# mantasu/face-crop-plus

Measured on AMD Instinct MI355X. Metric: faces/sec end-to-end (detect+align+crop), higher is better.
Workload: dtype f16x3; 1 GPU; RetinaFace detect + 5-pt align/crop, batch=32/GPU synthetic 1024x1024 RGB, strategy=largest, det_threshold=0.6, output 256x256, detector on 2 HIP streams x 16 images; global_batch=32, image_size=1024, parallelism=dp1

## Files before the change

face-crop-plus_amd/_native.py:

```python
from __future__ import annotations

import ctypes as C
import os

_HERE = os.path.dirname(os.path.abspath(__file__))
LIB_PATH = os.path.join(_HERE, "csrc", "libfcp_hip.so")
ABI_VERSION = 15

c_f32p = C.c_void_p
_lib = None


class ConvDesc(C.Structure):
    _fields_ = [
        ("in_", C.c_void_p), ("w", C.c_void_p), ("bias", C.c_void_p), ("out", C.c_void_p),
        ("res1", C.c_void_p), ("res2", C.c_void_p), ("wscale", C.c_void_p), ("in2", C.c_void_p),
        ("n", C.c_int32), ("in_h", C.c_int32), ("in_w", C.c_int32),
        ("cin", C.c_int32), ("in_ld", C.c_int32), ("in_up2", C.c_int32),
        ("cout", C.c_int32), ("kh", C.c_int32), ("kw", C.c_int32),
        ("stride", C.c_int32), ("pad", C.c_int32),
        ("out_h", C.c_int32), ("out_w", C.c_int32), ("out_ld", C.c_int32),
        ("tile_n", C.c_int32), ("cin4", C.c_int32),
        ("act_slope", C.c_float), ("alpha", C.c_float), ("alpha2", C.c_float),
        ("res1_pre", C.c_int32), ("res1_ld", C.c_int32), ("res1_h", C.c_int32),
# ... 5 lines not shown
    ]


CONV_FLAT_ADDR = 1
CONV_BALANCE_TAIL = 2
CHAIN_OUT_EVEN_ONLY = 1


class ChainDesc(C.Structure):
    _fields_ = [(k, C.c_void_p) for k in ("t1", "w2", "ws2", "b2", "w3", "ws3", "b3", "res", "out", "w1n", "ws1n",
                                          "b1n", "t1n", "t1b")] + \
               [(k, C.c_int32) for k in ("n", "h", "w", "c", "cn", "t1_ld", "res_ld", "out_ld", "t1n_ld", "nout", "tile_m", "flags",
                                         "cb", "t1b_ld", "t1b_h", "t1b_w", "t1b_stride")]


_P, _I, _F, _L = C.c_void_p, C.c_int, C.c_float, C.c_int64
SIGNATURES = {
    "fcp_conv2d_nhwc_f32": [C.POINTER(ConvDesc), _P],
    "fcp_bottleneck_chain_f16x3": [C.POINTER(ChainDesc), _P],
    "fcp_u8_to_nhwc4_f32": [_P, _P, _L, C.POINTER(C.c_float), _F, _P],
    "fcp_f32nchw_to_nhwc4_f32": [_P, _P, _I, _I, _I, C.POINTER(C.c_float), _F, _P],
    "fcp_maxpool3x3s2_nhwc_f32": [_P, _P, _I, _I, _I, _I, _I, _I, _I, _P],
    "fcp_maxpool3x3s2_split32": [_P, _P, _I, _I, _I, _I, _I, _I, _I, _P],
    "fcp_stem7x7s2_relu_pool_u8": [_P, _I, _I, _I, C.POINTER(C.c_int32), _P, _P, _P, _P, _I, _I, _P],
    "fcp_stem7x7s2_relu_pool_conv1_u8": [_P, _I, _I, _I, C.POINTER(C.c_int32), _P, _P, _P, _P, _I, _I, _P, _P, _P, _P, _I, _P],
    "fcp_stem7x7s2_relu_pool_f32": [_P, _I, _I, _I, _P, _P, _P, _P, _I, _I, _P],
    "fcp_f32_to_split32": [_P, _P, _L, _I, _P],
    "fcp_split32_to_f32": [_P, _P, _L, _I, _P],
    "fcp_absmax_nhwc": [_P, _L, _I, _I, _I, _P, _P],
    "fcp_retina_decode": [_P, _P, _P, _I, _I, _I, _F, _F, _F, _P, _P, _P, _P, _P, _P, _P, _P, _P],
    "fcp_retina_nms_select": [_P, _P, _P, _I, _I, _F, _I, _P, _P, _P, _P, _P, _P],
    "fcp_retina_gather_faces": [_P, _P, _P, _I, _I, _P, _I, _P, _P, _P, _P],
    "fcp_estimate_transform": [_P, _P, _I, _I, _I, _P, _P, _P],
    "fcp_estimate_transform_counted": [_P, _P, _I, _I, _I, _P, _P, _P, _P, _P],
# ... 116 lines not shown
```

face-crop-plus_amd/csrc/fcp_bneck_chain.hip:

```cpp
#include "fcp_conv_common.h"

#include <type_traits>

using namespace fcp_conv;

namespace {

constexpr int FCP_CHAIN_STORE_AUX = 2;

struct ChainK {
  const float* t1;  unsigned t1_bytes;  int t1_ld;
  const float* w2;  unsigned w2_bytes;  const float* ws2;  const float* b2;
  const float* w3;  unsigned w3_bytes;  const float* ws3;  const float* b3;
  const float* res; int res_ld;
  float* out;       int out_ld;    unsigned out_bytes;
  const float* w1n; unsigned w1n_bytes; const float* ws1n; const float* b1n;
  float* t1n;       int t1n_ld;
  int n, h, w, M;
  int nt_store;
  int out_even;
  const float* t1b; unsigned t1b_bytes; int t1b_ld, hb, wb, sb;
};

constexpr int BMT = 128;
// ... 2 lines not shown
constexpr int STAGE = (BMT + C) * ROWB;
constexpr int CT_OFF = 0;
constexpr int W1B_OFF = BMT * 128;
constexpr bool w1_double(int cn, bool has_c2) { return !has_c2 || W1B_OFF + 2 * cn * 128 + 2 * C * 128 <= 2 * STAGE; }
constexpr int w3b_off(int cn, bool has_c2) { return W1B_OFF + (w1_double(cn, has_c2) ? 2 : 1) * cn * 128; }
constexpr int r0_bytes(int cw, int cn, bool has_c2) { return has_c2 ? 2 * STAGE : w3b_off(cn, has_c2) + 2 * cw * 128; }
constexpr bool alias_t2(bool has_c2) { return !has_c2; }
constexpr int lds_bytes(int cw, int cn, bool has_c2, bool direct = false) {
  const int r0 = r0_bytes(cw, cn, has_c2), t2 = BMT * cw * 4;
  if (direct) return r0;
  return !alias_t2(has_c2) ? r0 + t2 : (r0 > W1B_OFF + t2 ? r0 : W1B_OFF + t2);
}
constexpr int wgs_per_cu(int cw, int cn, bool has_c2, bool direct = false) {
  if (direct) return cn == 0 && lds_bytes(cw, cn, has_c2, true) <= 80 * 1024 ? 2 : 1;
  return lds_bytes(cw, cn, has_c2) <= 80 * 1024 ? 2 : 1;
}

__device__ __forceinline__ void mfma3(f32x16& acc, const f16x8& ah, const f16x8& al, const f16x8& bh, const f16x8& bl) {
  acc = __builtin_amdgcn_mfma_f32_32x32x16_f16(al, bh, acc, 0, 0, 0);
  acc = __builtin_amdgcn_mfma_f32_32x32x16_f16(ah, bl, acc, 0, 0, 0);
  acc = __builtin_amdgcn_mfma_f32_32x32x16_f16(ah, bh, acc, 0, 0, 0);
}

__device__ __forceinline__ void row_values8(const float* c8, const float (&ws8)[8], const float (&b8)[8], float (&v)[8]) {
  const f32x4 a = *reinterpret_cast<const f32x4*>(c8);
  const f32x4 b = *reinterpret_cast<const f32x4*>(c8 + 4);
#pragma unroll
  for (int e = 0; e < 4; ++e) {
    v[e] = conv_value_relu(a[e], ws8[e], b8[e]);
    v[4 + e] = conv_value_relu(b[e], ws8[4 + e], b8[4 + e]);
  }
}

constexpr bool direct_form(int cn, int cw2) { return cw2 > 0 || cn == 0; }
template <int CN, int CW, int NOUT, bool HAS_C2, bool HAS_RES, int CW2 = 0>
__global__ void __launch_bounds__(2 * BMT, wgs_per_cu(CW, CN, HAS_C2, direct_form(CN, CW2))) bneck_chain_c64(const ChainK p) {
// ... 594 lines not shown
```

face-crop-plus_amd/csrc/fcp_conv_common.h:

```cpp
#pragma once
#include <type_traits>
#include "fcp_common.h"
#include "fcp_hip.h"

typedef float f32x16 __attribute__((ext_vector_type(16)));
typedef float f32x4 __attribute__((ext_vector_type(4)));


constexpr int FCP_AUX_A = 0;
constexpr int FCP_AUX_B = 0;

namespace fcp_conv {

constexpr int BM = 128;
constexpr int BK = 32;

struct ConvK {
  const float* in;
  const float* w;
  const float* bias;
  float* out;
  const float* res1;
  const float* res2;
  int n, in_h, in_w, ph, pw, cin, in_ld, in_up2;
// ... 175 lines not shown
template <int IMM>
__device__ __forceinline__ f16x8 lds_read128i(unsigned addr) {
  f16x8 v;
  asm volatile("ds_read_b128 %0, %1 offset:%2" : "=v"(v) : "v"(addr), "n"(IMM));
  return v;
}

template <int TM, int TN>
__device__ __forceinline__ void clear_acc(f32x16 (&acc)[TM][TN]) {
#pragma unroll
  for (int i = 0; i < TM; ++i)
#pragma unroll
    for (int j = 0; j < TN; ++j)
#pragma unroll
      for (int e = 0; e < 16; ++e) acc[i][j][e] = 0.f;
}

template <int HI>
__device__ __forceinline__ float fcp_mix_sum(unsigned h, unsigned l) {
  float r;
  const float one = 1.0f;
  if constexpr (HI) asm("v_fma_mix_f32 %0, %1, %2, %3 op_sel:[1,0,1] op_sel_hi:[1,0,1]" : "=v"(r) : "v"(h), "s"(one), "v"(l));
  else asm("v_fma_mix_f32 %0, %1, %2, %3 op_sel:[0,0,0] op_sel_hi:[1,0,1]" : "=v"(r) : "v"(h), "s"(one), "v"(l));
  return r;
}
template <int HI>
__device__ __forceinline__ float fcp_mix_diff(float x, unsigned h) {
  float r;
  const float minus_one = -1.0f;
  if constexpr (HI) asm("v_fma_mix_f32 %0, %1, %2, %3 op_sel:[1,0,0] op_sel_hi:[1,0,0]" : "=v"(r) : "v"(h), "s"(minus_one), "v"(x));
// ... 377 lines not shown
```

face-crop-plus_amd/csrc/torch_ops/fcp_torch_ops.cpp:

```cpp
#include <ATen/ATen.h>
#include <ATen/hip/HIPContext.h>
#include <c10/core/DeviceGuard.h>
#include <torch/library.h>

#include <climits>
#include <tuple>

#include "fcp_hip.h"

namespace {

using at::Tensor;

void* cur_stream() { return (void*)at::hip::getCurrentHIPStream().stream(); }

#define FCP_DEVICE_GUARD(t) const c10::OptionalDeviceGuard fcp_guard_(at::device_of(t))

void ok(int rc, const char* what) { TORCH_CHECK(rc == 0, what, " failed (", rc, "): ", fcp_last_error()); }

const Tensor& dev(const Tensor& t, const char* name, at::ScalarType dt) {
  TORCH_CHECK(t.is_cuda(), name, " must live on the GPU");
  TORCH_CHECK(t.scalar_type() == dt, name, " has dtype ", t.scalar_type(), ", expected ", dt);
  TORCH_CHECK(t.is_contiguous(), name, " must be contiguous");
  return t;
// ... 116 lines not shown
  } else {
    d.t1n = nullptr;
  }
  d.n = (int)t1.size(0); d.h = (int)t1.size(1); d.w = (int)t1.size(2); d.c = (int)c; d.cn = (int)cn; d.nout = (int)nout;
  d.t1_ld = (int)t1.size(3); d.out_ld = (int)nout; d.t1n_ld = (int)cn; d.tile_m = (int)tile_m; d.flags = (int)flags;
  if (two) {
    dev(*t1b, "t1b", at::kFloat);
    TORCH_CHECK(t1b->dim() == 4 && t1b->size(0) == t1.size(0) && t1b_c0 + cb <= t1b->size(3), "t1b (n,hb,wb,>=cb) split32 buffer");
    d.t1b = t1b->data_ptr<float>() + t1b_c0; d.cb = (int)cb; d.t1b_ld = (int)t1b->size(3);
    d.t1b_h = (int)t1b->size(1); d.t1b_w = (int)t1b->size(2); d.t1b_stride = (int)t1b_stride;
  }
  ok(fcp_bottleneck_chain_f16x3(&d, cur_stream()), "fcp::bottleneck_chain");
  return {out, t1n};
}

std::tuple<Tensor, Tensor, Tensor, Tensor, Tensor> retina_decode(const Tensor& h0, const Tensor& h1, const Tensor& h2,
                                                                 int64_t img_h, int64_t img_w, double vis, double var0,
                                                                 double var1) {
  dev(h0, "head0", at::kFloat); dev(h1, "head1", at::kFloat); dev(h2, "head2", at::kFloat);
  FCP_DEVICE_GUARD(h0);
  TORCH_CHECK(img_h > 0 && img_w > 0, "image size must be positive");
  TORCH_CHECK(h0.dim() == 4, "head maps are (n, ceil(h/s), ceil(w/s), 32) fp32 NHWC");
  const int64_t n = h0.size(0);
  int64_t P = 0;
  const Tensor* heads[3] = {&h0, &h1, &h2};
  int li = 0;
  for (int64_t s : {8, 16, 32}) {
    const Tensor& h = *heads[li++];
    const int64_t fh = (img_h + s - 1) / s, fw = (img_w + s - 1) / s;
    TORCH_CHECK(h.dim() == 4 && h.size(0) == n && h.size(1) == fh && h.size(2) == fw && h.size(3) == 32,
// ... 611 lines not shown

TORCH_LIBRARY(fcp, m) {
  m.def("conv2d(Tensor x, int x_c0, int cin, Tensor w, Tensor? bias, Tensor? wscale, Tensor? res1, int res1_c0, Tensor? res2, "
        "int res2_c0, int cout, int kh, int kw, int stride, int pad, float act_slope, float alpha, "
        "float alpha2, bool res1_pre, int precision, int in_fmt, int out_fmt, int res1_fmt, int res2_fmt, bool in_up2, "
        "bool cin4, int tile_m, int tile_n, Tensor? x2, int x2_c0, int cin2, int x2_stride, int flags, int cu_budget=0, int band_top=0, "
        "int band_bottom=0) -> Tensor");
  m.def("conv2d_out(Tensor x, int x_c0, int cin, Tensor w, Tensor? bias, Tensor? wscale, Tensor? res1, int res1_c0, Tensor? res2, "
        "int res2_c0, Tensor(a!) out, int out_c0, int cout, int kh, int kw, int stride, int pad, float act_slope, float alpha, "
        "float alpha2, bool res1_pre, int precision, int in_fmt, int out_fmt, int res1_fmt, int res2_fmt, bool in_up2, "
        "bool cin4, int tile_m, int tile_n, Tensor? x2, int x2_c0, int cin2, int x2_stride, int flags, int cu_budget=0, int band_top=0, "
        "int band_bottom=0) -> ()");
  m.def("bottleneck_chain(Tensor t1, int t1_c0, Tensor? res, int res_c0, Tensor? w2, Tensor? ws2, Tensor? b2, Tensor w3, Tensor ws3, "
        "Tensor b3, Tensor? w1n, Tensor? ws1n, Tensor? b1n, int c, int nout, int cn, int tile_m=0, int flags=0, Tensor? t1b=None, "
        "int t1b_c0=0, int cb=0, int t1b_stride=1) -> (Tensor, Tensor)");
  m.def("retina_decode(Tensor head0, Tensor head1, Tensor head2, int img_h, int img_w, float vis, float var0, float var1) "
        "-> (Tensor, Tensor, Tensor, Tensor, Tensor)");
  m.def("nms_select(Tensor cand_score, Tensor cand_box, Tensor cand_count, float nms_threshold, int strategy) "
        "-> (Tensor, Tensor, Tensor, Tensor)");
  m.def("gather_faces(Tensor cand_ldm, Tensor sel_pos, Tensor sel_count, Tensor? paddings, int max_faces) -> (Tensor, Tensor, Tensor)");
  m.def("similarity_from_5pt(Tensor src, Tensor dst, bool allow_skew, Tensor? face_count=None, Tensor(a!)? valid_total=None) "
        "-> (Tensor, Tensor)");
  m.def("warp_affine_u8(Tensor images, Tensor img_idx, Tensor mat, Tensor? ok, Tensor? paddings, int out_w, int out_h, int border) -> Tensor");
  m.def("warp_affine_u8_float(Tensor images, Tensor img_idx, Tensor mat, Tensor? ok, Tensor? paddings, int out_w, int out_h, "
        "int border) -> Tensor");
  m.def("warp_affine_u8_ragged(Tensor blob, Tensor srcs, Tensor mat, Tensor? ok, int out_w, int out_h, int border, int family) "
        "-> Tensor");
  m.def("warp_affine_u8_interp(Tensor images, Tensor img_idx, Tensor mat, Tensor? ok, Tensor? paddings, int out_w, int out_h, "
        "int border, int interp) -> Tensor");
  m.def("warp_affine_u8_interp_ragged(Tensor blob, Tensor srcs, Tensor mat, Tensor? ok, int out_w, int out_h, int border, "
// ... 21 lines not shown
  m.def("matte_image(Tensor crops, Tensor labels, int class_bits, int feather, Tensor pictures, Tensor picks, bool with_alpha) "
        "-> (Tensor, Tensor)");
  m.def("matte_image_alpha(Tensor crops, Tensor alpha, Tensor pictures, Tensor picks) -> Tensor");
  m.def("cutout_image(Tensor crops, Tensor alpha, Tensor pictures, Tensor picks, int[] taps) -> Tensor");
  m.def("bicubic_down4_round(Tensor x4) -> Tensor");
  m.def("parse_argmax_hist(Tensor logits, int ncls, int mid_h, int mid_w, int out_h, int out_w) -> (Tensor, Tensor)");
  m.def("abi_version() -> (int, int)", []() -> std::tuple<int64_t, int64_t> {
    return {(int64_t)FCP_ABI_VERSION, (int64_t)fcp_abi_version()};
  });
}

TORCH_LIBRARY_IMPL(fcp, CUDA, m) {
  m.impl("conv2d", &conv2d);
  m.impl("conv2d_out", &conv2d_out);
  m.impl("bottleneck_chain", &bottleneck_chain);
  m.impl("retina_decode", &retina_decode);
  m.impl("nms_select", &nms_select);
  m.impl("gather_faces", &gather_faces);
  m.impl("similarity_from_5pt", &similarity_from_5pt);
  m.impl("warp_affine_u8", &warp_affine_u8);
  m.impl("warp_affine_u8_float", &warp_affine_u8_float);
  m.impl("warp_affine_u8_ragged", &warp_affine_u8_ragged);
  m.impl("warp_affine_u8_interp", &warp_affine_u8_interp);
  m.impl("warp_affine_u8_interp_ragged", &warp_affine_u8_interp_ragged);
  m.impl("resize_area_u8_ragged", &resize_area_u8_ragged);
  m.impl("crop_sharpness", &crop_sharpness);
  m.impl("jpeg_encode", &jpeg_encode);
  m.impl("jpeg_encode_ex", &jpeg_encode_ex);
  m.impl("jpeg_huffman_tables", &jpeg_huffman_tables);
  m.impl("png_encode", &png_encode);
// ... 20 lines not shown
```

face-crop-plus_amd/engine.py:

```python
from __future__ import annotations

import contextlib
import ctypes as C
import os
import threading
from dataclasses import dataclass

import numpy as np
import torch

from . import _native as N
from . import torch_ops as T

BN_EPS = 1e-5
COUT_PAD = 128


class Act:
    __slots__ = ("buf", "c0", "c", "fmt")

    def __init__(self, buf: torch.Tensor, c0: int = 0, c: int | None = None, fmt: int = 0):
        assert buf.dim() == 4 and buf.dtype == torch.float32 and buf.is_contiguous()
        self.buf, self.c0, self.fmt = buf, c0, fmt
        self.c = buf.shape[3] - c0 if c is None else c
# ... 723 lines not shown
                    + c * nout + nout * cn)
        if pc1n is None:
            head = f"expand {c}->{nout} @{t1.h}x{t1.w}"
            return f"{head} +res", head, flops, byts
        head = f"chain {'3x3 ' if pc2 is not None else ''}{c}->{nout}->{cn} @{t1.h}x{t1.w}"
        return (f"{head}{' +res' if res is not None else ''}{' out@even' if flags else ''}{' two-source' if t1b is not None else ''}",
                head, flops, byts)

    def relaunch(o, o1n):
        o = _alias_safe_out(o, t1, res, t1b)
        o1n = o1n if o1n is None else _alias_safe_out(o1n, t1, res, t1b)
        return "fcp_bottleneck_chain_f16x3", (C.byref(desc(o, o1n)),), (pc2, pc3, pc1n, t1, res, o, o1n, t1b)
    return _accounted(go, describe, relaunch)


def u8_to_nhwc4(images_u8: torch.Tensor, sub=(0.0, 0.0, 0.0), div: float = 1.0) -> Act:
    assert images_u8.dtype == torch.uint8 and images_u8.dim() == 4 and images_u8.shape[3] == 3
    assert images_u8.is_contiguous()
    n, h, w, _ = images_u8.shape
    out = Act.empty(n, h, w, 4, images_u8.device)
    sub_arr = (C.c_float * 3)(*[float(s) for s in sub])
    N.check(N.lib().fcp_u8_to_nhwc4_f32(N.ptr(images_u8), out.ptr(), n * h * w, sub_arr, float(div),
                                        N.stream_ptr()), "fcp_u8_to_nhwc4_f32")
    return out


@dataclass
class PackedStem:
    wfrag: torch.Tensor
    bias: torch.Tensor
# ... 137 lines not shown
```

face-crop-plus_amd/retinaface.py:

```python
from __future__ import annotations


import os
import threading

import numpy as np
import torch

from . import _native as N
from . import engine as E
from . import torch_ops as T
from .weights import load_state_dict

STRATEGIES = {"all": 0, "best": 1, "largest": 2}


class RetinaFace:
    WEIGHTS_FILENAME = "retinaface_detector.pth"

    def __init__(self, strategy: str = "all", vis: float = 0.6):
        self.strategy = strategy
        self.vis_threshold = vis
        self.nms_threshold = 0.4
        self.variance = [0.1, 0.2]
        self.device = None
        self._p = None
        self.precision = 0
        self.fused_chain = True
        self.streams = int(os.environ.get("FCP_DET_STREAMS", "2"))
        self.min_images_per_stream = 6
        self._tls = threading.local()

    def load(self, device: str | torch.device = "cuda:0", weights=None, precision=None):
        device = torch.device(device)
        if device.type != "cuda":
            raise RuntimeError("face_crop_plus_amd runs on an AMD GPU only (device must be cuda:N / hip); "
                               "there is no CPU fallback")
        N.lib()
        self.device = device
        sd = load_state_dict("retinaface", weights, device=device)
        self._repack(sd, precision)
        E.device_props(device)
        E.selfcheck_at_load(self, sd, weights, precision, lambda: self._repack(sd, "f32"))
# ... 142 lines not shown
                if blk["feat"]:
                    feats.append(x)
                continue
            idt = x if blk["ds"] is None else E.conv(blk["ds"], x, out_fmt=f)
            x = E.conv(blk["c3"], o, act_slope=0.0, res1=idt, res1_pre=True, out_fmt=f)
            if blk["feat"]:
                feats.append(x)
        if getattr(self, "_debug_feats", None) is not None:
            self._debug_feats.extend(feats)
        o3 = E.conv(p["fpn.output3"], feats[2], act_slope=0.0, out_fmt=f)
        o2 = E.conv(p["fpn.output2"], feats[1], act_slope=0.0, res1=o3, res1_pre=False, out_fmt=f)
        o2 = E.conv(p["fpn.merge2"], o2, act_slope=0.0, out_fmt=f)
        o1 = E.conv(p["fpn.output1"], feats[0], act_slope=0.0, res1=o2, res1_pre=False, out_fmt=f)
        o1 = E.conv(p["fpn.merge1"], o1, act_slope=0.0, out_fmt=f)
        heads = []
        for k, ft in zip((1, 2, 3), (o1, o2, o3)):
            s = E.Act.empty(ft.n, ft.h, ft.w, 384, ft.buf.device, f)
            E.conv(p[f"ssh{k}.ab"], ft, s.slice(0, 192), act_slope=0.0)
            E.conv(p[f"ssh{k}.cd"], s.slice(0, 64), s.slice(256, 128), act_slope=0.0)
            E.conv(p[f"ssh{k}.e"], s.slice(320, 64), s.slice(192, 64), act_slope=0.0)
            heads.append(E.conv(p[f"head{k}"], s.slice(64, 256),
                                None if heads_out is None else heads_out[k - 1]))
        return heads

    def _side_streams(self, dev, k):
        main = E.thread_streams(dev)["main"]
        return E.thread_side_streams(dev, k, with_main=main is not None and torch.cuda.current_stream(dev) == main)

    MAX_OPERAND_BYTES = 0xFFFFFFF0

    def _images_per_launch(self, h: int, w: int) -> int | None:
# ... 177 lines not shown
```

face-crop-plus_amd/torch_ops.py:

```python
from __future__ import annotations

import os

import torch

_HERE = os.path.dirname(os.path.abspath(__file__))
LIB_PATH = os.path.join(_HERE, "csrc", "libfcp_torch.so")
_loaded = False


def _default_enabled() -> bool:
    mode = os.environ.get("FCP_BOUNDARY", "auto").lower()
    if mode == "ctypes":
        return False
    if mode == "torch":
        return True
    if os.path.isfile(LIB_PATH):
        return True
    import warnings
    warnings.warn(f"{LIB_PATH} is missing (the torch.ops.fcp veneer was not built): calling the C ABI through ctypes")
    return False


ENABLED = _default_enabled()
# ... 3 lines not shown
    global _loaded
    if not _loaded:
        if not os.path.isfile(LIB_PATH):
            raise RuntimeError(f"torch op library not built: {LIB_PATH} is missing "
                               f"(run `python face-crop-plus_amd/build_native.py`)")
        torch.ops.load_library(LIB_PATH)
        from ._native import ABI_VERSION
        built, running = torch.ops.fcp.abi_version()
        if built != ABI_VERSION or running != ABI_VERSION:
            raise RuntimeError(f"libfcp_torch.so is stale: compiled against ABI {built}, libfcp_hip.so reports {running}, "
                               f"host code expects {ABI_VERSION}; rebuild (python face-crop-plus_amd/build_native.py --force)")
        _loaded = True
    return torch.ops.fcp


OPS = ("conv2d", "conv2d_out", "bottleneck_chain", "retina_decode", "nms_select", "gather_faces", "similarity_from_5pt",
       "warp_affine_u8", "warp_affine_u8_float", "warp_affine_u8_ragged", "resize_area_u8_ragged", "bicubic_down4_round",
       "parse_argmax_hist", "warp_affine_u8_interp", "warp_affine_u8_interp_ragged", "crop_sharpness", "jpeg_encode", "matte", "clahe", "matte_blur",
       "jpeg_encode_ex", "jpeg_huffman_tables", "matte_refine", "matte_alpha", "matte_blur_alpha",
       "subject_mask", "png_encode", "png_huffman_lengths", "feather_alpha", "cutout", "mask_shift", "nlm_denoise", "unsharp",
       "matte_image", "matte_image_alpha", "cutout_image")
```

include/fcp_hip.h:

```cpp
#ifndef FCP_HIP_H
#define FCP_HIP_H

#include <stdint.h>

#ifdef __cplusplus
extern "C" {
#endif

#define FCP_ABI_VERSION 15

typedef void* fcp_stream_t;

int fcp_abi_version(void);
const char* fcp_last_error(void);

typedef struct fcp_conv_desc {
  const float* in;
  const void* w;
  const float* bias;
  float* out;
  const float* res1;
  const float* res2;
  const float* wscale;
  const float* in2;
// ... 28 lines not shown
  float* out;
  const void* w1n; const float* ws1n; const float* b1n;
  float* t1n;
  const float* t1b;
  int32_t n, h, w, c, cn;
  int32_t t1_ld, res_ld, out_ld, t1n_ld;
  int32_t nout;
  int32_t tile_m;
  int32_t flags;
  int32_t cb, t1b_ld, t1b_h, t1b_w, t1b_stride;
} fcp_chain_desc;
#define FCP_CHAIN_OUT_EVEN_ONLY 1

int fcp_bottleneck_chain_f16x3(const fcp_chain_desc* desc, fcp_stream_t stream);

int fcp_u8_to_nhwc4_f32(const uint8_t* in, float* out, int64_t npix,
                        const float* sub_host, float div, fcp_stream_t stream);

int fcp_f32nchw_to_nhwc4_f32(const float* in, float* out, int n, int h, int w,
                             const float* sub_host, float div, fcp_stream_t stream);

int fcp_maxpool3x3s2_nhwc_f32(const float* in, float* out, int n, int h, int w, int c, int out_ld,
                              int out_h, int out_w, fcp_stream_t stream);
int fcp_maxpool3x3s2_split32(const float* in, float* out, int n, int h, int w, int c, int out_ld,
                             int out_h, int out_w, fcp_stream_t stream);
int fcp_stem7x7s2_relu_pool_u8(const uint8_t* images, int n, int h, int w, const int32_t* mean_rgb,
                               const void* wfrag, const float* bias, const float* wscale, float* out,
                               int out_ld, int out_fmt, fcp_stream_t stream);
int fcp_stem7x7s2_relu_pool_conv1_u8(const uint8_t* images, int n, int h, int w, const int32_t* mean_rgb,
                                     const void* wfrag, const float* bias, const float* wscale, float* out,
// ... 202 lines not shown
```

Baseline: 1459 faces/s.

## Fuse SSH context convolutions and detection head into one tiled kernel

Adds a fused HIP kernel that, per 8x16 pixel tile with halo, runs the SSH cd 3x3 conv, the e 3x3 conv and the 1x1 head conv, keeping all intermediates in LDS. Previously these ran as separate launches that wrote and re-read a 384-channel intermediate buffer. The tile recomputes the cd conv over a halo region, which adds redundant FLOPs, and the kernel uses one workgroup per CU with a large LDS footprint. It is enabled only for small feature maps (up to 40x40) in split32 precision mode.

```diff
diff --git a/face-crop-plus_amd/_native.py b/face-crop-plus_amd/_native.py
--- a/face-crop-plus_amd/_native.py
+++ b/face-crop-plus_amd/_native.py
@@ -43,10 +43,17 @@
                                          "cb", "t1b_ld", "t1b_h", "t1b_w", "t1b_stride")]
 
 
+class SshTailDesc(C.Structure):
+    _fields_ = [(k, C.c_void_p) for k in ("b", "a", "w_cd", "ws_cd", "b_cd", "w_e", "ws_e", "b_e", "w_head", "ws_head",
+                                          "b_head", "out")] + \
+               [(k, C.c_int32) for k in ("n", "h", "w", "b_ld", "a_ld", "out_ld")]
+
+
 _P, _I, _F, _L = C.c_void_p, C.c_int, C.c_float, C.c_int64
 SIGNATURES = {
     "fcp_conv2d_nhwc_f32": [C.POINTER(ConvDesc), _P],
     "fcp_bottleneck_chain_f16x3": [C.POINTER(ChainDesc), _P],
+    "fcp_ssh_tail_f16x3": [C.POINTER(SshTailDesc), _P],
     "fcp_u8_to_nhwc4_f32": [_P, _P, _L, C.POINTER(C.c_float), _F, _P],
     "fcp_f32nchw_to_nhwc4_f32": [_P, _P, _I, _I, _I, C.POINTER(C.c_float), _F, _P],
     "fcp_maxpool3x3s2_nhwc_f32": [_P, _P, _I, _I, _I, _I, _I, _I, _I, _P],
diff --git a/face-crop-plus_amd/csrc/fcp_bneck_chain.hip b/face-crop-plus_amd/csrc/fcp_bneck_chain.hip
--- a/face-crop-plus_amd/csrc/fcp_bneck_chain.hip
+++ b/face-crop-plus_amd/csrc/fcp_bneck_chain.hip
@@ -40,12 +40,6 @@
 constexpr int wgs_per_cu(int cw, int cn, bool has_c2, bool direct = false) {
   if (direct) return cn == 0 && lds_bytes(cw, cn, has_c2, true) <= 80 * 1024 ? 2 : 1;
   return lds_bytes(cw, cn, has_c2) <= 80 * 1024 ? 2 : 1;
-}
-
-__device__ __forceinline__ void mfma3(f32x16& acc, const f16x8& ah, const f16x8& al, const f16x8& bh, const f16x8& bl) {
-  acc = __builtin_amdgcn_mfma_f32_32x32x16_f16(al, bh, acc, 0, 0, 0);
-  acc = __builtin_amdgcn_mfma_f32_32x32x16_f16(ah, bl, acc, 0, 0, 0);
-  acc = __builtin_amdgcn_mfma_f32_32x32x16_f16(ah, bh, acc, 0, 0, 0);
 }
 
 __device__ __forceinline__ void row_values8(const float* c8, const float (&ws8)[8], const float (&b8)[8], float (&v)[8]) {
diff --git a/face-crop-plus_amd/csrc/fcp_conv_common.h b/face-crop-plus_amd/csrc/fcp_conv_common.h
--- a/face-crop-plus_amd/csrc/fcp_conv_common.h
+++ b/face-crop-plus_amd/csrc/fcp_conv_common.h
@@ -213,6 +213,12 @@
     for (int j = 0; j < TN; ++j)
 #pragma unroll
       for (int e = 0; e < 16; ++e) acc[i][j][e] = 0.f;
+}
+
+__device__ __forceinline__ void mfma3(f32x16& acc, const f16x8& ah, const f16x8& al, const f16x8& bh, const f16x8& bl) {
+  acc = __builtin_amdgcn_mfma_f32_32x32x16_f16(al, bh, acc, 0, 0, 0);
+  acc = __builtin_amdgcn_mfma_f32_32x32x16_f16(ah, bl, acc, 0, 0, 0);
+  acc = __builtin_amdgcn_mfma_f32_32x32x16_f16(ah, bh, acc, 0, 0, 0);
 }
 
 template <int HI>
diff --git a/face-crop-plus_amd/csrc/fcp_ssh_tail.hip b/face-crop-plus_amd/csrc/fcp_ssh_tail.hip
--- /dev/null
+++ b/face-crop-plus_amd/csrc/fcp_ssh_tail.hip
@@ -0,0 +1,331 @@
+#include "fcp_conv_common.h"
+
+#include <type_traits>
+
+using namespace fcp_conv;
+
+namespace {
+
+struct TailK {
+  const float* b;   unsigned b_bytes;  int b_ld;
+  const float* a;   unsigned a_bytes;  int a_ld;
+  const float* wcd; const float* wscd; const float* bcd;
+  const float* we;  const float* wse;  const float* be;
+  const float* wh;  const float* wsh;  const float* bh;
+  float* out;       int out_ld;
+  int n, h, w;
+};
+
+constexpr int ROWB = 128;
+constexpr int PH = 8, PW = 16, PIX = PH * PW;
+constexpr int BH = PH + 4, BW = PW + 4, BROWS = BH * BW;
+constexpr int DH = PH + 2, DW = PW + 2, DROWS = DH * DW;
+constexpr int DT = (DROWS + 31) / 32;
+constexpr int CK = 64;
+constexpr int KT = 9 * CK / BK;
+constexpr int WROW3 = 9 * CK * 4;
+constexpr int HK = 256, HS = HK / BK, HN = 32;
+constexpr int B_OFF = 0, B_SL = BROWS * ROWB;
+constexpr int D_OFF = 0, D_SL = DROWS * ROWB;
+constexpr int E_OFF = 0, E_SL = PIX * ROWB;
+constexpr int RCD_OFF = B_OFF + 2 * B_SL, RCD_ST = 128 * ROWB;
+constexpr int C_OFF = RCD_OFF, C_SL = PIX * ROWB;
+constexpr int RE_OFF = RCD_OFF + 2 * RCD_ST, RE_ST = 64 * ROWB;
+constexpr int WH_OFF = RE_OFF + 2 * RE_ST, WH_SL = HN * ROWB;
+constexpr int LDS_BYTES = WH_OFF + HS * WH_SL;
+static_assert(2 * D_SL <= 2 * B_SL && 2 * E_SL <= 2 * D_SL && 2 * C_SL <= 2 * RCD_ST, "the aliased images must fit the regions they reuse");
+static_assert(DT * 32 / 2 == 96 && LDS_BYTES <= 160 * 1024, "wave tiles / LDS budget");
+
+__device__ __forceinline__ void put2(char* a0, char* a1, unsigned v) {
+  *reinterpret_cast<unsigned short*>(a0) = (unsigned short)(v & 0xFFFFu);
+  *reinterpret_cast<unsigned short*>(a1) = (unsigned short)(v >> 16);
+}
+__device__ __forceinline__ int img_hi(int row, int c) { return row * ROWB + (((c >> 3) ^ swz(row)) << 4) + (c & 7) * 2; }
+__device__ __forceinline__ int img_lo(int row, int c) { return row * ROWB + (((4 + (c >> 3)) ^ swz(row)) << 4) + (c & 7) * 2; }
+
+__global__ void __launch_bounds__(256, 1) ssh_tail_f16x3(const TailK p) {
+  extern __shared__ __attribute__((aligned(16))) float smem[];
+  char* lds = reinterpret_cast<char*>(smem);
+  const int tile = xcd_tile_order(gridDim.x, blockIdx.x);
+  const int tid = threadIdx.x;
+  const int lane = tid & 63;
+  const int wave = tid >> 6;
+  const int wave_u = __builtin_amdgcn_readfirstlane(wave);
+  const int l31 = lane & 31, half = lane >> 5;
+  const int wm = wave_u >> 1, wn = wave_u & 1;
+  int offH[2], offL[2];
+  frag_offsets(lane, offH, offL);
+  auto frag_pair = [&](const char* row, int s, f16x8& hi, f16x8& lo) {
+    hi = *reinterpret_cast<const f16x8*>(row + offH[s]);
+    lo = *reinterpret_cast<const f16x8*>(row + offL[s]);
+  };
+  auto frag_pair_at = [&](const char* img, int row, int s, f16x8& hi, f16x8& lo) {
+    const int sw = swz(row);
+    hi = *reinterpret_cast<const f16x8*>(img + row * ROWB + (((2 * s + half) ^ sw) << 4));
+    lo = *reinterpret_cast<const f16x8*>(img + row * ROWB + (((4 + 2 * s + half) ^ sw) << 4));
+  };
+  const int txn = (p.w + PW - 1) / PW, tyn = (p.h + PH - 1) / PH;
+  const int tr = tile / txn;
+  const int px0 = (tile - tr * txn) * PW;
+  const int pn = tr / tyn;
+  const int py0 = (tr - pn * tyn) * PH;
+  auto inside = [&](int y, int x) { return (unsigned)y < (unsigned)p.h && (unsigned)x < (unsigned)p.w; };
+
+  __amdgpu_buffer_rsrc_t rs_b = __builtin_amdgcn_make_buffer_rsrc(const_cast<float*>(p.b), 0, p.b_bytes, 0x00020000);
+  __amdgpu_buffer_rsrc_t rs_a = __builtin_amdgcn_make_buffer_rsrc(const_cast<float*>(p.a), 0, p.a_bytes, 0x00020000);
+  __amdgpu_buffer_rsrc_t rs_wcd = __builtin_amdgcn_make_buffer_rsrc(const_cast<float*>(p.wcd), 0, 128u * WROW3, 0x00020000);
+  __amdgpu_buffer_rsrc_t rs_we = __builtin_amdgcn_make_buffer_rsrc(const_cast<float*>(p.we), 0, 64u * WROW3, 0x00020000);
+  __amdgpu_buffer_rsrc_t rs_wh = __builtin_amdgcn_make_buffer_rsrc(const_cast<float*>(p.wh), 0, (unsigned)(HN * HK * 4), 0x00020000);
+
+#pragma unroll
+  for (int i = 0; i < (BROWS / 8 + 3) / 4; ++i) {
+    const int g = wave_u + 4 * i;
+    if (g < BROWS / 8) {
+      const int r = 8 * g + (lane >> 3);
+      const int hy = r / BW, hx = r - hy * BW;
+      const int y = py0 - 2 + hy, x = px0 - 2 + hx;
+      const unsigned src = inside(y, x) ? (unsigned)((pn * p.h + y) * p.w + x) * (unsigned)p.b_ld * 4u + (unsigned)(((lane & 7) ^ swz(r)) << 4) : 0xFFFFFFFFu;
+#pragma unroll
+      for (int cs = 0; cs < 2; ++cs)
+        __builtin_amdgcn_raw_ptr_buffer_load_lds(rs_b, (__attribute__((address_space(3))) void*)(lds + B_OFF + cs * B_SL + g * 8 * ROWB), 16,
+                                                 (int)(src == 0xFFFFFFFFu ? 0xFFFFFFFFu : src + (unsigned)(cs * 128)), 0, 0, FCP_AUX_A);
+    }
+  }
+#pragma unroll
+  for (int i = 0; i < HS * (HN / 8) / 4; ++i) {
+    const int q = wave_u * (HS * (HN / 8) / 4) + i, sl = q >> 2, g = q & 3;
+    const int r = 8 * g + (lane >> 3);
+    __builtin_amdgcn_raw_ptr_buffer_load_lds(rs_wh, (__attribute__((address_space(3))) void*)(lds + WH_OFF + sl * WH_SL + g * 8 * ROWB), 16,
+                                             (int)(unsigned)(r * (HK * 4) + sl * 128 + (((lane & 7) ^ swz(r)) << 4)), 0, 0, FCP_AUX_B);
+  }
+  f16x8 aah[4][2], aal[4][2];
+  {
+    const int pp = wave * 32 + l31;
+    const int y = py0 + (pp >> 4), x = px0 + (pp & 15);
+    const unsigned base = inside(y, x) ? (unsigned)((pn * p.h + y) * p.w + x) * (unsigned)p.a_ld * 4u : 0xFFFFFFFFu;
+#pragma unroll
+    for (int sl = 0; sl < 4; ++sl)
+#pragma unroll
+      for (int s = 0; s < 2; ++s) {
+        const unsigned vh = base == 0xFFFFFFFFu ? base : base + (unsigned)(sl * 128 + ((2 * s + half) << 4));
+        const unsigned vl = base == 0xFFFFFFFFu ? base : base + (unsigned)(sl * 128 + ((4 + 2 * s + half) << 4));
+        aah[sl][s] = __builtin_bit_cast(f16x8, __builtin_amdgcn_raw_buffer_load_b128(rs_a, (int)vh, 0, 0));
+        aal[sl][s] = __builtin_bit_cast(f16x8, __builtin_amdgcn_raw_buffer_load_b128(rs_a, (int)vl, 0, 0));
+      }
+  }
+
+  auto dma_piece = [&](__amdgpu_buffer_rsrc_t rs, int ring_off, int stage_bytes, int rows_per_wave, int kt) {
+#pragma unroll
+    for (int i = 0; i < 4; ++i) {
+      if (i < rows_per_wave / 8) {
+        const int g = wave_u * (rows_per_wave / 8) + i;
+        const int r = 8 * g + (lane >> 3);
+        __builtin_amdgcn_raw_ptr_buffer_load_lds(rs, (__attribute__((address_space(3))) void*)(lds + ring_off + (kt & 1) * stage_bytes + g * 8 * ROWB), 16,
+                                                 (int)(unsigned)(r * WROW3 + kt * 128 + (((lane & 7) ^ swz(r)) << 4)), 0, 0, FCP_AUX_B);
+      }
+    }
+  };
+
+  {
+    f32x16 acc[3][2];
+    clear_acc(acc);
+    int hrow[3];
+#pragma unroll
+    for (int i = 0; i < 3; ++i) {
+      const int r0 = (3 * wm + i) * 32 + l31;
+      const int r = r0 < DROWS ? r0 : DROWS - 1;
+      const int ry = r / DW;
+      hrow[i] = ry * BW + (r - ry * DW);
+    }
+    const char* Bw = lds + RCD_OFF + (wn * 64 + l31) * ROWB;
+    dma_piece(rs_wcd, RCD_OFF, RCD_ST, 32, 0);
+    fcp_static_for<0, KT>([&](auto kc) {
+      constexpr int kt = decltype(kc)::value, cs = kt / 9, tap = kt % 9;
+      asm volatile("s_waitcnt vmcnt(0)" ::: "memory");
+      __builtin_amdgcn_s_barrier();
+      __builtin_amdgcn_sched_barrier(0);
+      f16x8 ah[2][3], al[2][3], bh[2][2], bl[2][2];
+#pragma unroll
+      for (int s = 0; s < 2; ++s) {
+#pragma unroll
+        for (int i = 0; i < 3; ++i) frag_pair_at(lds + B_OFF + cs * B_SL, hrow[i] + (tap / 3) * BW + tap % 3, s, ah[s][i], al[s][i]);
+#pragma unroll
+        for (int j = 0; j < 2; ++j) frag_pair(Bw + (kt & 1) * RCD_ST + j * 32 * ROWB, s, bh[s][j], bl[s][j]);
+      }
+      __builtin_amdgcn_sched_barrier(0);
+      if constexpr (kt + 1 < KT) dma_piece(rs_wcd, RCD_OFF, RCD_ST, 32, kt + 1);
+      __builtin_amdgcn_sched_barrier(0);
+#pragma unroll
+      for (int s = 0; s < 2; ++s)
+#pragma unroll
+        for (int i = 0; i < 3; ++i)
+#pragma unroll
+          for (int j = 0; j < 2; ++j) mfma3(acc[i][j], ah[s][i], al[s][i], bh[s][j], bl[s][j]);
+      __builtin_amdgcn_sched_barrier(0);
+    });
+    asm volatile("s_waitcnt vmcnt(0)" ::: "memory");
+    __builtin_amdgcn_s_barrier();
+    __builtin_amdgcn_sched_barrier(0);
+    float ws[2], bb[2];
+#pragma unroll
+    for (int j = 0; j < 2; ++j) {
+      ws[j] = p.wscd[wn * 64 + j * 32 + l31];
+      bb[j] = p.bcd[wn * 64 + j * 32 + l31];
+    }
+    auto cd_epilogue = [&](auto is_d) {
+      constexpr bool IS_D = decltype(is_d)::value;
+      char* img = lds + (IS_D ? D_OFF : C_OFF);
+      constexpr int SL = IS_D ? D_SL : C_SL;
+#pragma unroll
+      for (int i = 0; i < 3; ++i)
+#pragma unroll
+        for (int q = 0; q < 8; ++q) {
+          int oh[2], ol[2];
+          bool zero[2];
+#pragma unroll
+          for (int e = 0; e < 2; ++e) {
+            const int r = (3 * wm + i) * 32 + mfma_c_row(2 * q + e, half);
+            const int ry = r / DW, rx = r - ry * DW;
+            const int row = IS_D ? r : (ry - 1) * PW + (rx - 1);
+            const bool keep = IS_D ? r < DROWS : (ry >= 1 && ry <= PH && rx >= 1 && rx <= PW);
+            zero[e] = IS_D && !inside(py0 - 1 + ry, px0 - 1 + rx);
+            oh[e] = keep ? img_hi(row, l31) : -1;
+            ol[e] = keep ? img_lo(row, l31) : -1;
+          }
+#pragma unroll
+          for (int j = 0; j < 2; ++j) {
+            float v[2];
+#pragma unroll
+            for (int e = 0; e < 2; ++e) {
+              v[e] = conv_value_relu(acc[i][j][2 * q + e], ws[j], bb[j]);
+              if (zero[e]) v[e] = 0.f;
+            }
+            unsigned hu, lu;
+            split2(v[0], v[1], hu, lu);
+#pragma unroll
+            for (int e = 0; e < 2; ++e)
+              if (oh[e] >= 0) {
+                *reinterpret_cast<unsigned short*>(img + j * SL + oh[e]) = (unsigned short)(e ? hu >> 16 : hu & 0xFFFFu);
+                *reinterpret_cast<unsigned short*>(img + j * SL + ol[e]) = (unsigned short)(e ? lu >> 16 : lu & 0xFFFFu);
+              }
+          }
+        }
+    };
+    if (wn == 1) cd_epilogue(std::true_type{});
+    else cd_epilogue(std::false_type{});
+    __syncthreads();
+  }
+
+  {
+    f32x16 acc[2][1];
+    clear_acc(acc);
+    int drow[2];
+#pragma unroll
+    for (int i = 0; i < 2; ++i) {
+      const int pp = (2 * wm + i) * 32 + l31;
+      drow[i] = (pp >> 4) * DW + (pp & 15);
+    }
+    const char* Bw = lds + RE_OFF + (wn * 32 + l31) * ROWB;
+    dma_piece(rs_we, RE_OFF, RE_ST, 16, 0);
+    fcp_static_for<0, KT>([&](auto kc) {
+      constexpr int kt = decltype(kc)::value, cs = kt / 9, tap = kt % 9;
+      asm volatile("s_waitcnt vmcnt(0)" ::: "memory");
+      __builtin_amdgcn_s_barrier();
+      __builtin_amdgcn_sched_barrier(0);
+      f16x8 ah[2][2], al[2][2], bh[2], bl[2];
+#pragma unroll
+      for (int s = 0; s < 2; ++s) {
+#pragma unroll
+        for (int i = 0; i < 2; ++i) frag_pair_at(lds + D_OFF + cs * D_SL, drow[i] + (tap / 3) * DW + tap % 3, s, ah[s][i], al[s][i]);
+        frag_pair(Bw + (kt & 1) * RE_ST, s, bh[s], bl[s]);
+      }
+      __builtin_amdgcn_sched_barrier(0);
+      if constexpr (kt + 1 < KT) dma_piece(rs_we, RE_OFF, RE_ST, 16, kt + 1);
+      __builtin_amdgcn_sched_barrier(0);
+#pragma unroll
+      for (int s = 0; s < 2; ++s)
+#pragma unroll
+        for (int i = 0; i < 2; ++i) mfma3(acc[i][0], ah[s][i], al[s][i], bh[s], bl[s]);
+      __builtin_amdgcn_sched_barrier(0);
+    });
+    asm volatile("s_waitcnt vmcnt(0)" ::: "memory");
+    __builtin_amdgcn_s_barrier();
+    __builtin_amdgcn_sched_barrier(0);
+    const float ws = p.wse[wn * 32 + l31], bb = p.be[wn * 32 + l31];
+    char* img = lds + E_OFF + wn * E_SL;
+#pragma unroll
+    for (int i = 0; i < 2; ++i)
+#pragma unroll
+      for (int q = 0; q < 8; ++q) {
+        const int r0 = (2 * wm + i) * 32 + mfma_c_row(2 * q, half), r1 = (2 * wm + i) * 32 + mfma_c_row(2 * q + 1, half);
+        unsigned hu, lu;
+        split2(conv_value_relu(acc[i][0][2 * q], ws, bb), conv_value_relu(acc[i][0][2 * q + 1], ws, bb), hu, lu);
+        put2(img + img_hi(r0, l31), img + img_hi(r1, l31), hu);
+        put2(img + img_lo(r0, l31), img + img_lo(r1, l31), lu);
+      }
+    __syncthreads();
+  }
+
+  {
+    f32x16 acc;
+#pragma unroll
+    for (int e = 0; e < 16; ++e) acc[e] = 0.f;
+    const char* Wh = lds + WH_OFF + l31 * ROWB;
+    const int prow = (wave * 32 + l31) * ROWB;
+#pragma unroll
+    for (int sl = 0; sl < HS; ++sl)
+#pragma unroll
+      for (int s = 0; s < 2; ++s) {
+        f16x8 ah, al, bh, bl;
+        if (sl < 4) {
+          ah = aah[sl][s];
+          al = aal[sl][s];
+        } else {
+          frag_pair(lds + (sl < 6 ? E_OFF + (sl - 4) * E_SL : C_OFF + (sl - 6) * C_SL) + prow, s, ah, al);
+        }
+        frag_pair(Wh + sl * WH_SL, s, bh, bl);
+        mfma3(acc, ah, al, bh, bl);
+      }
+    const float ws = p.wsh[l31], bb = p.bh[l31];
+    const ConvEpi epi = {false, false, false, 1.f, 1.f, 1.f};
+#pragma unroll
+    for (int rr = 0; rr < 16; ++rr) {
+      const int pp = wave * 32 + mfma_c_row(rr, half);
+      const int y = py0 + (pp >> 4), x = px0 + (pp & 15);
+      if (inside(y, x)) p.out[((long)(pn * p.h + y) * p.w + x) * p.out_ld + l31] = conv_value(epi, acc[rr], ws, bb, 0.f, 0.f);
+    }
+  }
+}
+
+}
+
+extern "C" int fcp_ssh_tail_f16x3(const fcp_ssh_tail_desc* d, fcp_stream_t stream) {
+  FCP_REQUIRE(d != nullptr, "ssh tail: null descriptor");
+  FCP_REQUIRE(d->b && d->a && d->out, "ssh tail: null tensor");
+  FCP_REQUIRE(d->w_cd && d->ws_cd && d->b_cd && d->w_e && d->ws_e && d->b_e && d->w_head && d->ws_head && d->b_head,
+              "ssh tail: null filter (every convolution carries a bias and filter scales)");
+  FCP_REQUIRE(d->n > 0 && d->h > 0 && d->w > 0, "ssh tail: bad sizes");
+  const long M = (long)d->n * d->h * d->w;
+  FCP_REQUIRE(M < (1L << 31), "ssh tail: too many pixels");
+  auto aligned = [](const void* p, int ld) { return ((uintptr_t)p & 127) == 0 && ld % 32 == 0; };
+  FCP_REQUIRE(aligned(d->b, d->b_ld) && aligned(d->a, d->a_ld), "ssh tail: b and a are split32 views: 128-byte aligned, channel stride a multiple of 32");
+  FCP_REQUIRE(d->b_ld >= CK && d->a_ld >= 128 && d->out_ld >= HN, "ssh tail: channel strides too small (b 64, a 128, out 32 channels)");
+  FCP_REQUIRE(((uintptr_t)d->out & 3) == 0, "ssh tail: out must be 4-byte aligned");
+  FCP_REQUIRE((((uintptr_t)d->w_cd | (uintptr_t)d->w_e | (uintptr_t)d->w_head) & 15) == 0, "ssh tail: filters must be 16-byte aligned");
+  const unsigned long b_bytes = ((unsigned long)(M - 1) * d->b_ld + CK) * 4ul, a_bytes = ((unsigned long)(M - 1) * d->a_ld + 128) * 4ul;
+  FCP_REQUIRE(b_bytes < 0xFFFFFFF0ul && a_bytes < 0xFFFFFFF0ul, "ssh tail: b and a must span less than 4 GiB each");
+  TailK k;
+  k.b = d->b; k.b_bytes = (unsigned)b_bytes; k.b_ld = d->b_ld;
+  k.a = d->a; k.a_bytes = (unsigned)a_bytes; k.a_ld = d->a_ld;
+  k.wcd = reinterpret_cast<const float*>(d->w_cd); k.wscd = d->ws_cd; k.bcd = d->b_cd;
+  k.we = reinterpret_cast<const float*>(d->w_e); k.wse = d->ws_e; k.be = d->b_e;
+  k.wh = reinterpret_cast<const float*>(d->w_head); k.wsh = d->ws_head; k.bh = d->b_head;
+  k.out = d->out; k.out_ld = d->out_ld;
+  k.n = d->n; k.h = d->h; k.w = d->w;
+  const long tiles = (long)d->n * fcp_cdiv(d->h, PH) * fcp_cdiv(d->w, PW);
+  FCP_REQUIRE(tiles < (1L << 31), "ssh tail: too many patches");
+  FCP_LDS_OPT_IN(&ssh_tail_f16x3, LDS_BYTES);
+  hipLaunchKernelGGL(ssh_tail_f16x3, dim3((unsigned)tiles), dim3(256), LDS_BYTES, (hipStream_t)stream, k);
+  FCP_LAUNCH_OK();
+  return 0;
+}
diff --git a/face-crop-plus_amd/csrc/torch_ops/fcp_torch_ops.cpp b/face-crop-plus_amd/csrc/torch_ops/fcp_torch_ops.cpp
--- a/face-crop-plus_amd/csrc/torch_ops/fcp_torch_ops.cpp
+++ b/face-crop-plus_amd/csrc/torch_ops/fcp_torch_ops.cpp
@@ -154,6 +154,27 @@
   return {out, t1n};
 }
 
+void ssh_tail_out(const Tensor& s, int64_t s_c0, const Tensor& w_cd, const Tensor& ws_cd, const Tensor& b_cd, const Tensor& w_e,
+                  const Tensor& ws_e, const Tensor& b_e, const Tensor& w_head, const Tensor& ws_head, const Tensor& b_head,
+                  Tensor& out, int64_t out_c0) {
+  dev(s, "s", at::kFloat);
+  FCP_DEVICE_GUARD(s);
+  dev(out, "out", at::kFloat);
+  TORCH_CHECK(s.dim() == 4 && s_c0 >= 0 && s_c0 + 192 <= s.size(3), "s (n,h,w,>=192) split32 buffer holding [B | A]");
+  TORCH_CHECK(out.dim() == 4 && out.size(0) == s.size(0) && out.size(1) == s.size(1) && out.size(2) == s.size(2) && out_c0 >= 0 &&
+              out_c0 + 32 <= out.size(3), "out has the wrong geometry");
+  for (const Tensor* w : {&w_cd, &w_e, &w_head}) TORCH_CHECK(w->is_cuda() && w->is_contiguous(), "filters must be contiguous GPU tensors (packed)");
+  fcp_ssh_tail_desc d = {};
+  d.b = s.data_ptr<float>() + s_c0; d.a = d.b + 64; d.out = out.data_ptr<float>() + out_c0;
+  d.w_cd = w_cd.data_ptr(); d.ws_cd = dev(ws_cd, "ws_cd", at::kFloat).data_ptr<float>(); d.b_cd = dev(b_cd, "b_cd", at::kFloat).data_ptr<float>();
+  d.w_e = w_e.data_ptr(); d.ws_e = dev(ws_e, "ws_e", at::kFloat).data_ptr<float>(); d.b_e = dev(b_e, "b_e", at::kFloat).data_ptr<float>();
+  d.w_head = w_head.data_ptr(); d.ws_head = dev(ws_head, "ws_head", at::kFloat).data_ptr<float>();
+  d.b_head = dev(b_head, "b_head", at::kFloat).data_ptr<float>();
+  d.n = (int)s.size(0); d.h = (int)s.size(1); d.w = (int)s.size(2);
+  d.b_ld = d.a_ld = (int)s.size(3); d.out_ld = (int)out.size(3);
+  ok(fcp_ssh_tail_f16x3(&d, cur_stream()), "fcp::ssh_tail_out");
+}
+
 std::tuple<Tensor, Tensor, Tensor, Tensor, Tensor> retina_decode(const Tensor& h0, const Tensor& h1, const Tensor& h2,
                                                                  int64_t img_h, int64_t img_w, double vis, double var0,
                                                                  double var1) {
@@ -795,6 +816,8 @@
   m.def("bottleneck_chain(Tensor t1, int t1_c0, Tensor? res, int res_c0, Tensor? w2, Tensor? ws2, Tensor? b2, Tensor w3, Tensor ws3, "
         "Tensor b3, Tensor? w1n, Tensor? ws1n, Tensor? b1n, int c, int nout, int cn, int tile_m=0, int flags=0, Tensor? t1b=None, "
         "int t1b_c0=0, int cb=0, int t1b_stride=1) -> (Tensor, Tensor)");
+  m.def("ssh_tail_out(Tensor s, int s_c0, Tensor w_cd, Tensor ws_cd, Tensor b_cd, Tensor w_e, Tensor ws_e, Tensor b_e, Tensor w_head, "
+        "Tensor ws_head, Tensor b_head, Tensor(a!) out, int out_c0) -> ()");
   m.def("retina_decode(Tensor head0, Tensor head1, Tensor head2, int img_h, int img_w, float vis, float var0, float var1) "
         "-> (Tensor, Tensor, Tensor, Tensor, Tensor)");
   m.def("nms_select(Tensor cand_score, Tensor cand_box, Tensor cand_count, float nms_threshold, int strategy) "
@@ -846,6 +869,7 @@
   m.impl("conv2d", &conv2d);
   m.impl("conv2d_out", &conv2d_out);
   m.impl("bottleneck_chain", &bottleneck_chain);
+  m.impl("ssh_tail_out", &ssh_tail_out);
   m.impl("retina_decode", &retina_decode);
   m.impl("nms_select", &nms_select);
   m.impl("gather_faces", &gather_faces);
diff --git a/face-crop-plus_amd/engine.py b/face-crop-plus_amd/engine.py
--- a/face-crop-plus_amd/engine.py
+++ b/face-crop-plus_amd/engine.py
@@ -761,6 +761,58 @@
     return _accounted(go, describe, relaunch)
 
 
+SSH_TAIL_MAX_MAP = 40 * 40
+
+
+def ssh_tail_supported(pc_cd: PackedConv, pc_e: PackedConv, pc_head: PackedConv, map_hw: tuple[int, int] | None = None) -> bool:
+    convs = (pc_cd, pc_e, pc_head)
+    if not all(pc is not None and pc.precision == 1 and pc.bias is not None and not pc.cin4 for pc in convs):
+        return False
+    shape = lambda pc: (pc.cin, pc.cout, pc.kh, pc.kw, pc.stride, pc.pad)
+    if (shape(pc_cd), shape(pc_e), shape(pc_head)) != ((64, 128, 3, 3, 1, 1), (64, 64, 3, 3, 1, 1), (256, 32, 1, 1, 1, 0)):
+        return False
+    return map_hw is None or map_hw[0] * map_hw[1] <= SSH_TAIL_MAX_MAP
+
+
+def _ssh_tail_desc(pc_cd, pc_e, pc_head, b: Act, a: Act, out: Act) -> N.SshTailDesc:
+    d = N.SshTailDesc()
+    d.b, d.a, d.out = b.ptr(), a.ptr(), out.ptr()
+    d.w_cd, d.ws_cd, d.b_cd = map(N.ptr, _filter(pc_cd))
+    d.w_e, d.ws_e, d.b_e = map(N.ptr, _filter(pc_e))
+    d.w_head, d.ws_head, d.b_head = map(N.ptr, _filter(pc_head))
+    d.n, d.h, d.w = b.n, b.h, b.w
+    d.b_ld, d.a_ld, d.out_ld = b.ld, a.ld, out.ld
+    return d
+
+
+def ssh_tail(pc_cd: PackedConv, pc_e: PackedConv, pc_head: PackedConv, s_ab: Act, head_out: Act | None = None) -> Act:
+    assert ssh_tail_supported(pc_cd, pc_e, pc_head), "ssh_tail: unsupported shapes"
+    assert s_ab.fmt == 1 and s_ab.c == 192, "ssh_tail reads the split32 [B | A] view of the ab conv"
+    b, a = s_ab.slice(0, 64), s_ab.slice(64, 128)
+    if head_out is None:
+        head_out = Act.empty(b.n, b.h, b.w, pc_head.cout, b.buf.device, 0)
+    assert head_out.fmt == 0 and (head_out.n, head_out.h, head_out.w, head_out.c) == (b.n, b.h, b.w, pc_head.cout), "ssh_tail: bad output view"
+
+    def go():
+        if T.ENABLED:
+            T.load().ssh_tail_out(s_ab.buf, s_ab.c0, *_filter(pc_cd), *_filter(pc_e), *_filter(pc_head), head_out.buf, head_out.c0)
+        else:
+            _c_launch("fcp_ssh_tail_f16x3", C.byref(_ssh_tail_desc(pc_cd, pc_e, pc_head, b, a, head_out)))
+        return (head_out,)
+
+    def describe():
+        m = b.n * b.h * b.w
+        patches = b.n * -(-b.h // 8) * -(-b.w // 16)
+        flops = (pc_cd.flops_per_pixel + pc_e.flops_per_pixel + pc_head.flops_per_pixel) * m + pc_cd.flops_per_pixel * patches * (180 - 128)
+        byts = 4 * (m * (64 + 128 + pc_head.cout) + 9 * 64 * (128 + 64) + 256 * pc_head.cout)
+        label = f"ssh tail 64->128|64->{pc_head.cout} @{b.h}x{b.w}"
+        return label, label, flops, byts
+
+    def relaunch(o):
+        return "fcp_ssh_tail_f16x3", (C.byref(_ssh_tail_desc(pc_cd, pc_e, pc_head, b, a, o)),), (pc_cd, pc_e, pc_head, s_ab, o)
+    return _accounted(go, describe, relaunch)[0]
+
+
 def u8_to_nhwc4(images_u8: torch.Tensor, sub=(0.0, 0.0, 0.0), div: float = 1.0) -> Act:
     assert images_u8.dtype == torch.uint8 and images_u8.dim() == 4 and images_u8.shape[3] == 3
     assert images_u8.is_contiguous()
diff --git a/face-crop-plus_amd/retinaface.py b/face-crop-plus_amd/retinaface.py
--- a/face-crop-plus_amd/retinaface.py
+++ b/face-crop-plus_amd/retinaface.py
@@ -27,6 +27,7 @@
         self._p = None
         self.precision = 0
         self.fused_chain = True
+        self.fused_ssh_tail = True
         self.streams = int(os.environ.get("FCP_DET_STREAMS", "2"))
         self.min_images_per_stream = 6
         self._tls = threading.local()
@@ -199,7 +200,14 @@
         o1 = E.conv(p["fpn.output1"], feats[0], act_slope=0.0, res1=o2, res1_pre=False, out_fmt=f)
         o1 = E.conv(p["fpn.merge1"], o1, act_slope=0.0, out_fmt=f)
         heads = []
+        tail = bool(f) and self.fused_ssh_tail and E.RangeMonitor.active is None
         for k, ft in zip((1, 2, 3), (o1, o2, o3)):
+            ho = None if heads_out is None else heads_out[k - 1]
+            if tail and E.ssh_tail_supported(p[f"ssh{k}.cd"], p[f"ssh{k}.e"], p[f"head{k}"], (ft.h, ft.w)):
+                s = E.Act.empty(ft.n, ft.h, ft.w, 192, ft.buf.device, f)
+                E.conv(p[f"ssh{k}.ab"], ft, s, act_slope=0.0)
+                heads.append(E.ssh_tail(p[f"ssh{k}.cd"], p[f"ssh{k}.e"], p[f"head{k}"], s, ho))
+                continue
             s = E.Act.empty(ft.n, ft.h, ft.w, 384, ft.buf.device, f)
             E.conv(p[f"ssh{k}.ab"], ft, s.slice(0, 192), act_slope=0.0)
             E.conv(p[f"ssh{k}.cd"], s.slice(0, 64), s.slice(256, 128), act_slope=0.0)
diff --git a/face-crop-plus_amd/torch_ops.py b/face-crop-plus_amd/torch_ops.py
--- a/face-crop-plus_amd/torch_ops.py
+++ b/face-crop-plus_amd/torch_ops.py
@@ -41,7 +41,7 @@
     return torch.ops.fcp
 
 
-OPS = ("conv2d", "conv2d_out", "bottleneck_chain", "retina_decode", "nms_select", "gather_faces", "similarity_from_5pt",
+OPS = ("conv2d", "conv2d_out", "bottleneck_chain", "ssh_tail_out", "retina_decode", "nms_select", "gather_faces", "similarity_from_5pt",
        "warp_affine_u8", "warp_affine_u8_float", "warp_affine_u8_ragged", "resize_area_u8_ragged", "bicubic_down4_round",
        "parse_argmax_hist", "warp_affine_u8_interp", "warp_affine_u8_interp_ragged", "crop_sharpness", "jpeg_encode", "matte", "clahe", "matte_blur",
        "jpeg_encode_ex", "jpeg_huffman_tables", "matte_refine", "matte_alpha", "matte_blur_alpha",
diff --git a/include/fcp_hip.h b/include/fcp_hip.h
--- a/include/fcp_hip.h
+++ b/include/fcp_hip.h
@@ -66,6 +66,19 @@
 
 int fcp_bottleneck_chain_f16x3(const fcp_chain_desc* desc, fcp_stream_t stream);
 
+typedef struct fcp_ssh_tail_desc {
+  const float* b;
+  const float* a;
+  const void* w_cd;   const float* ws_cd;   const float* b_cd;
+  const void* w_e;    const float* ws_e;    const float* b_e;
+  const void* w_head; const float* ws_head; const float* b_head;
+  float* out;
+  int32_t n, h, w;
+  int32_t b_ld, a_ld, out_ld;
+} fcp_ssh_tail_desc;
+
+int fcp_ssh_tail_f16x3(const fcp_ssh_tail_desc* desc, fcp_stream_t stream);
+
 int fcp_u8_to_nhwc4_f32(const uint8_t* in, float* out, int64_t npix,
                         const float* sub_host, float div, fcp_stream_t stream);
 
```

Result: no change. 1458 faces/s (-0.1%).
